# jketterl/digiham

Hardware: AMD Instinct MI355X
Metric: concurrent 48 kS/s DMR channels sustained end-to-end (rrc_filter->gfsk_demodulator->dmr_decoder) (higher is better)
Workload: dtype f32; 1 GPU; 16384 DMR channels/GPU x 3.96 s (190080 samples) of 48 kS/s FM-discriminator audio, full chain rrc(wide)->gfsk(10)->dmr_decoder incl. BPTC(196,96) (BASELINE con; channels_per_gpu=16384, total_channels=16384

## Files before the change

digiham_amd/csrc/dh_portable.hpp:

```cpp
#pragma once

#include <stdint.h>
#include <stddef.h>

#if defined(__HIPCC__) || defined(__HIP__)
#include <hip/hip_runtime.h>
#define DH_DEVICE_BUILD 1
#define DH_HD __host__ __device__ __forceinline__
#define DH_D __device__ __forceinline__
#else
#define DH_DEVICE_BUILD 0
#define DH_HD inline
#define DH_D inline
#endif

#if DH_DEVICE_BUILD && defined(__HIP_DEVICE_COMPILE__)
#define DH_ON_GPU 1
#else
#define DH_ON_GPU 0
#endif

#if DH_ON_GPU
#define DH_GPU_ELSE(gpu, cpu) gpu
#else
#define DH_GPU_ELSE(gpu, cpu) cpu
#endif

#define DH_WAVE 64

#if DH_ON_GPU
static __device__ __forceinline__ int dh_fresh_lane_id_() { int l = (int) threadIdx.x; asm volatile("" : "+v"(l)); return l; }
#define DH_FOR_LANES(lane) for (int lane = (int) threadIdx.x, dh_once_ = 1; dh_once_; dh_once_ = 0)
#define DH_FOR_LANES_FRESH(lane) for (int lane = dh_fresh_lane_id_(), dh_once_ = 1; dh_once_; dh_once_ = 0)
#define DH_BARRIER() do { __builtin_amdgcn_fence(__ATOMIC_RELEASE, "workgroup", "local"); __builtin_amdgcn_s_barrier(); \
                          __builtin_amdgcn_fence(__ATOMIC_ACQUIRE, "workgroup", "local"); } while (0)
#define DH_BALLOT_ACC(mask, pred, lane) (mask) = __builtin_amdgcn_ballot_w64((bool) (pred))
#else
#define DH_FOR_LANES(lane) for (int lane = 0; lane < DH_WAVE; ++lane)
#define DH_FOR_LANES_FRESH(lane) DH_FOR_LANES(lane)
#define DH_BARRIER() ((void) 0)
#define DH_BALLOT_ACC(mask, pred, lane) (mask) |= ((uint64_t) ((pred) ? 1 : 0) << (lane))
#endif
#define DH_IS_LANE0(lane) ((lane) == 0)
DH_HD bool dh_is_writer_lane() { return DH_GPU_ELSE(threadIdx.x == 0, true); }

DH_HD uint32_t dh_uniform(uint32_t x) { return DH_GPU_ELSE((uint32_t) __builtin_amdgcn_readfirstlane((int) x), x); }

DH_HD uint32_t dh_agent_load(const uint32_t* p) { return DH_GPU_ELSE(__hip_atomic_load(p, __ATOMIC_RELAXED, __HIP_MEMORY_SCOPE_AGENT), *p); }
DH_HD bool dh_agent_cas(uint32_t* p, uint32_t& seen, uint32_t want) {
#if DH_ON_GPU
    return __hip_atomic_compare_exchange_strong(p, &seen, want, __ATOMIC_RELAXED, __ATOMIC_RELAXED, __HIP_MEMORY_SCOPE_AGENT);
#else
    if (*p == seen) { *p = want; return true; }
    seen = *p;
    return false;
#endif
}
DH_HD void dh_agent_add(uint32_t* p, uint32_t v) { DH_GPU_ELSE(__hip_atomic_fetch_add(p, v, __ATOMIC_RELAXED, __HIP_MEMORY_SCOPE_AGENT), *p += v); }
DH_HD uint32_t dh_xcc_id() { return DH_GPU_ELSE(__builtin_amdgcn_s_getreg((31 << 11) | 20) & 15u, 0u); }
#if DH_ON_GPU
__device__ __forceinline__ void dh_nap() { __builtin_amdgcn_s_sleep(64); }
__device__ __forceinline__ void dh_acquire_behind_flag() { __builtin_amdgcn_fence(__ATOMIC_ACQUIRE, "agent"); __builtin_amdgcn_s_dcache_inv(); }
__device__ __forceinline__ void dh_release_before_flag() { asm volatile("s_waitcnt vmcnt(0) lgkmcnt(0)" ::: "memory"); __builtin_amdgcn_fence(__ATOMIC_RELEASE, "workgroup"); }
__device__ __forceinline__ uint32_t dh_opaque_scalar(uint32_t x) { asm volatile("" : "+s"(x)); return x; }
__device__ __forceinline__ void dh_barrier_global() { __syncthreads(); }
#else
inline void dh_nap() {}
inline void dh_acquire_behind_flag() {}
inline void dh_release_before_flag() {}
inline uint32_t dh_opaque_scalar(uint32_t x) { return x; }
inline void dh_barrier_global() {}
#endif

DH_HD int dh_popc32(uint32_t x) { return DH_GPU_ELSE(__popc(x), __builtin_popcount(x)); }
DH_HD int dh_popc64(uint64_t x) { return DH_GPU_ELSE(__popcll(x), __builtin_popcountll(x)); }
// ... 179 lines not shown
```

digiham_amd/csrc/dsp_core.hpp:

```cpp
#pragma once

#include "dh_portable.hpp"
#include "wave_ops.hpp"

#define DH_VARIANCE_SYMBOLS 100
#define DH_VOLUME_RB_SIZE 100
#define DH_FTILE 1024
#define DH_FIR_L 16
#define DH_PF_N 5
#define DH_PF_SINK 512
#define DH_MAX_NZ 160
#define DH_MAX_SPS 40
DH_HD uint32_t dh_history(uint32_t sps) { return DH_VARIANCE_SYMBOLS * (sps > 10u ? sps : 10u) + 152u; }
DH_HD uint32_t dh_tail_max(uint32_t sps) { return 256u + dh_history(sps); }
#define DH_STATE_HDR 32

enum { DH_ST_K = 0, DH_ST_OFF = 1, DH_ST_TAIL = 2, DH_ST_NSYM = 3, DH_ST_ORDERED = 4, DH_ST_BLOCKS = 5,
       DH_ST_P0 = 6,
       DH_ST_CUR_START = 7, DH_ST_CUR_OFF = 8, DH_ST_PREV_START = 9, DH_ST_PREV_OFF = 10,
       DH_ST_BLOCK_FLAGS = 11,
       DH_ST_E_CUR = 12, DH_ST_E_PREV = 13, DH_ST_E_COUNT = 14, DH_ST_E_BLOCK = 15,
       DH_ST_UNCERTAIN = 16, DH_ST_EXACT_RUNS = 17, DH_ST_EXACT_BLOCKS = 18,
       DH_ST_PART = 19,
       DH_ST_DIAG = 20 };
// ... 353 lines not shown
    return ok;
}
inline float dh_f16_error_coefficient(const DhF16Taps& F, uint32_t nz, double gain) {
    const double u = 5.9604644775390625e-08;
    const double ks = (double) F.ksteps, nref = 2.0 + (double) nz;
    const double mfma = F.one_chain ? 82.0 * ks * F.l1_g1 * (1.0 + 1.0 / 2048.0) + 41.0 * ks / 2048.0 * (3.0 * F.l1_g2 * (1.0 + 1.0 / 2048.0) + F.l1_g1)
                                    : 41.0 * ks * F.l1_g1 * (1.0 + 1.0 / 2048.0) + 82.0 * ks / 2048.0 * (F.l1_g2 + 0.5 * F.l1_g1);
    const double kl1 = (nref + 0.01) * F.l1 + 1.0001 * F.l1 + mfma
                     + 2.0 * (0.5 * F.l1_g2 / 4194304.0 + F.sum_delta * (1.0 + 1.0 / 4096.0) + u * F.l1) / u + (F.one_chain ? 2.1 : 3.1) * F.l1;
    const double coef = 1.44 * kl1 * u / (gain < 0 ? -gain : gain) * 1.0001;
    float f = (float) coef;
    if ((double) f < coef) { union { float f; uint32_t u; } b; b.f = f; b.u++; f = b.f; }
    return f;
}

#if DH_ON_GPU
template <int NZ, bool ONE>
__device__ __forceinline__ void dh_fir_f16(const float* hw, const dh_u4 (&G)[2 * DH_F16_KSTEPS_OF(NZ)], int lane, float k1, float k2, float* out16) {
    constexpr int DH_F16_KSTEPS = DH_F16_KSTEPS_OF(NZ), DH_F16_FRAGS = 2 * DH_F16_KSTEPS, DH_F16_H2_OFFSET = DH_F16_H2_OFFSET_OF(NZ);
    const int m = lane & 15, q = lane >> 4;
    const char* base = reinterpret_cast<const char*>(hw) + 32 * (int) DH_F16_ROW_BLOCK(m) + 16 * q;
    dh_h8 g[DH_F16_FRAGS];
#pragma unroll
    for (int f = 0; f < DH_F16_FRAGS; f++) g[f] = __builtin_bit_cast(dh_h8, G[f]);
#pragma unroll
    for (int TT = 0; TT < 4; TT += 2) {
        dh_h8 a1[2][DH_F16_KSTEPS], a2[2][DH_F16_KSTEPS];
#pragma unroll
        for (int t = 0; t < 2; t++)
#pragma unroll
            for (int s = 0; s < DH_F16_KSTEPS; s++) a1[t][s] = *reinterpret_cast<const dh_h8*>(base + 512 * (TT + t) + 64 * s);
        if constexpr (ONE) {
            dh_f32x4 acc[2] = { { 0.0f, 0.0f, 0.0f, 0.0f }, { 0.0f, 0.0f, 0.0f, 0.0f } };
#pragma unroll
            for (int s = 0; s < DH_F16_KSTEPS; s++)
#pragma unroll
                for (int t = 0; t < 2; t++) acc[t] = __builtin_amdgcn_mfma_f32_16x16x32_f16(a1[t][s], g[DH_F16_KSTEPS + s], acc[t], 0, 0, 0);
#pragma unroll
            for (int s = 0; s < DH_F16_KSTEPS; s++) {
#pragma unroll
                for (int t = 0; t < 2; t++) acc[t] = __builtin_amdgcn_mfma_f32_16x16x32_f16(a1[t][s], g[s], acc[t], 0, 0, 0);
#pragma unroll
                for (int t = 0; t < 2; t++) a2[t][s] = *reinterpret_cast<const dh_h8*>(base + 512 * (TT + t) + 64 * s + 4 * DH_F16_H2_OFFSET);
            }
#pragma unroll
            for (int s = 0; s < DH_F16_KSTEPS; s++)
#pragma unroll
                for (int t = 0; t < 2; t++) acc[t] = __builtin_amdgcn_mfma_f32_16x16x32_f16(a2[t][s], g[s], acc[t], 0, 0, 0);
#pragma unroll
            for (int t = 0; t < 2; t++)
#pragma unroll
                for (int r = 0; r < 4; r++) out16[4 * (TT + t) + r] = acc[t][r] * k1;
            __builtin_amdgcn_sched_group_barrier(0x100, 2 * DH_F16_KSTEPS, 0);
            __builtin_amdgcn_sched_group_barrier(0x008, 2 * DH_F16_KSTEPS, 0);
#pragma unroll
            for (int s = 0; s < DH_F16_KSTEPS; s++) { __builtin_amdgcn_sched_group_barrier(0x008, 2, 0); __builtin_amdgcn_sched_group_barrier(0x100, 2, 0); }
            __builtin_amdgcn_sched_group_barrier(0x008, 2 * DH_F16_KSTEPS, 0);
            (void) k2;
        } else {
            dh_f32x4 mn[2] = { { 0.0f, 0.0f, 0.0f, 0.0f }, { 0.0f, 0.0f, 0.0f, 0.0f } }, sc[2] = { { 0.0f, 0.0f, 0.0f, 0.0f }, { 0.0f, 0.0f, 0.0f, 0.0f } };
#pragma unroll
            for (int s = 0; s < DH_F16_KSTEPS; s++) {
#pragma unroll
                for (int t = 0; t < 2; t++) sc[t] = __builtin_amdgcn_mfma_f32_16x16x32_f16(a1[t][s], g[DH_F16_KSTEPS + s], sc[t], 0, 0, 0);
#pragma unroll
                for (int t = 0; t < 2; t++) mn[t] = __builtin_amdgcn_mfma_f32_16x16x32_f16(a1[t][s], g[s], mn[t], 0, 0, 0);
#pragma unroll
                for (int t = 0; t < 2; t++) a2[t][s] = *reinterpret_cast<const dh_h8*>(base + 512 * (TT + t) + 64 * s + 4 * DH_F16_H2_OFFSET);
            }
#pragma unroll
            for (int s = 0; s < DH_F16_KSTEPS; s++)
#pragma unroll
                for (int t = 0; t < 2; t++) sc[t] = __builtin_amdgcn_mfma_f32_16x16x32_f16(a2[t][s], g[s], sc[t], 0, 0, 0);
#pragma unroll
            for (int t = 0; t < 2; t++)
#pragma unroll
                for (int r = 0; r < 4; r++) out16[4 * (TT + t) + r] = __builtin_fmaf(sc[t][r], k2, mn[t][r] * k1);
// ... 17 lines not shown
        for (int i = 0; i < 3; i++) {
            const int pass = ONE ? (i == 0 ? 1 : i == 1 ? 0 : 2) : i;
            for (int s = 0; s < DH_F16_KSTEPS; s++) for (int qq = 0; qq < 4; qq++) for (int j = 0; j < 8; j++) {
                const int kk = 8 * qq + j;
                const uint32_t w = G[(pass == 1 ? DH_F16_KSTEPS : 0) + s][16 * qq + n][j >> 1];
                const float tap = dh_f16_value((uint16_t) (w >> (16 * (j & 1))));
                const uint16_t hv = (pass == 2 ? h2 : h1)[b16 + 32u * (uint32_t) s + (uint32_t) kk];
                if (pass == 0 && !ONE) mn = __builtin_fmaf(dh_f16_value(hv), tap, mn); else sc = __builtin_fmaf(dh_f16_value(hv), tap, sc);
            }
        }
        out16[4 * T + r] = ONE ? sc * k1 : __builtin_fmaf(sc, k2, mn * k1);
    }
}
#endif

DH_HD float dh_virtual_sample(const float* tail, uint32_t tc, const float* in, uint32_t idx) {
    return idx < tc ? tail[idx] : in[idx - tc];
}

struct DhAgcPair { float mn0, mx0, mn1, mx1; };

#if DH_ON_GPU
__device__ __forceinline__ void dh_agc_scan(DhDspShared& S, uint32_t k0, uint32_t k1, DH_LANE_STRUCT_REF(DhAgcPair, agc)) {
    const int lane = dh_fresh_lane_id_();
    const uint32_t e0 = 2u * (uint32_t) lane, e1 = e0 + 1u;
    const float c0 = e0 < k0 ? S.vol_old[e0] : S.vol_new[e0];
    const float c1 = e1 < k0 ? S.vol_old[e1] : S.vol_new[e1];
    const bool v0 = e0 < k1, v1 = e1 < k1;
    const float pmn0 = v0 ? c0 : DH_FLT_MAX, pmn1 = v1 ? c1 : DH_FLT_MAX;
    const float pmx0 = v0 ? c0 : DH_FLT_MIN, pmx1 = v1 ? c1 : DH_FLT_MIN;
    float pmn = dh_vmin(pmn0, pmn1), pmx = dh_vmax(pmx0, pmx1);
    const uint32_t r0 = 126u - e0, r1 = r0 + 1u;
    const float o0 = S.vol_old[r0], o1 = S.vol_old[r1];
    const float omn0 = r0 < DH_VOLUME_RB_SIZE ? o0 : DH_FLT_MAX, omn1 = r1 < DH_VOLUME_RB_SIZE ? o1 : DH_FLT_MAX;
    const float omx0 = r0 < DH_VOLUME_RB_SIZE ? o0 : DH_FLT_MIN, omx1 = r1 < DH_VOLUME_RB_SIZE ? o1 : DH_FLT_MIN;
    float smn = dh_vmin(omn0, omn1), smx = dh_vmax(omx0, omx1);
    dh_wave_prefix_minmax2(pmn, pmx, smn, smx);
    float epmn = DH_FLT_MAX, epmx = DH_FLT_MIN, esmn = DH_FLT_MAX, esmx = DH_FLT_MIN;
    dh_wave_prev4(epmn, epmx, esmn, esmx, pmn, pmx, smn, smx);
    const int from = (63 - lane) << 2;
    const float s1n = __int_as_float(__builtin_amdgcn_ds_bpermute(from, __float_as_int(esmn)));
    const float s1x = __int_as_float(__builtin_amdgcn_ds_bpermute(from, __float_as_int(esmx)));
    const float s0n = __int_as_float(__builtin_amdgcn_ds_bpermute(from, __float_as_int(dh_vmin(omn1, esmn))));
    const float s0x = __int_as_float(__builtin_amdgcn_ds_bpermute(from, __float_as_int(dh_vmax(omx1, esmx))));
    DhAgcPair r;
    r.mn0 = dh_vmin(dh_vmin(epmn, pmn0), s0n); r.mx0 = dh_vmax(dh_vmax(epmx, pmx0), s0x);
    r.mn1 = dh_vmin(pmn, s1n); r.mx1 = dh_vmax(pmx, s1x);
    S.mn[e0] = r.mn0; S.mx[e0] = r.mx0; S.mn[e1] = r.mn1; S.mx[e1] = r.mx1;
    agc = r;
}
#else
inline void dh_agc_scan(DhDspShared& S, uint32_t k0, uint32_t k1, DH_LANE_STRUCT_REF(DhAgcPair, agc)) {
    float pmn = DH_FLT_MAX, pmx = DH_FLT_MIN;
    for (uint32_t j = 0; j < k0; j++) { pmn = dh_fmin_(pmn, S.vol_old[j]); pmx = dh_fmax_(pmx, S.vol_old[j]); }
    for (uint32_t k = k0; k < k1; k++) {
        pmn = dh_fmin_(pmn, S.vol_new[k]); pmx = dh_fmax_(pmx, S.vol_new[k]);
        float smn = DH_FLT_MAX, smx = DH_FLT_MIN;
        for (uint32_t j = k + 1; j < DH_VOLUME_RB_SIZE; j++) { smn = dh_fmin_(smn, S.vol_old[j]); smx = dh_fmax_(smx, S.vol_old[j]); }
        S.mn[k] = dh_fmin_(pmn, smn); S.mx[k] = dh_fmax_(pmx, smx);
    }
    for (uint32_t l = 0; l < DH_WAVE; l++) {
        const uint32_t e0 = 2u * l, e1 = e0 + 1u, a = e0 >= k0 && e0 < k1 ? e0 : k0, b = e1 >= k0 && e1 < k1 ? e1 : k0;
        agc[l] = DhAgcPair{ S.mn[a], S.mx[a], S.mn[b], S.mx[b] };
    }
}
#endif

template <int NZ, bool FAST, int SPS> struct DhIsBounded {
// ... 211 lines not shown
                        const uint32_t c = e / nj;
                        jj = e - c * nj;
                        uint64_t m = rows & all;
                        for (uint32_t b = 0; b < c; b++) m &= m - 1;
                        i = (uint32_t) dh_ffs64(m);
                    }
                    const uint32_t j = j0 + jj;
                    const int32_t f = C.cur_start + (int32_t) (j * sps) + (j ? C.cur_off : 0) + (int32_t) i;
                    S.var_rb[i * DH_VARIANCE_SYMBOLS + j] = dh_exact_filtered_lds<NZ>(stage, base, C.nv, C.tapsf, C.gain, C.rgain, f);
                }
            }
        }
    }
    DH_BARRIER();
}

template <int NZ>
DH_COLD void dh_exact_fir_pass(const DhDspParams& P, DhDspShared& S, uint32_t need, DH_LANE_ARRAY(float, (&fo), DH_FIR_L)) {
    float tv[NZ / 2 + 1];
    for (int i = 0; i <= NZ / 2; i++) tv[i] = S.tapsf[i];
    DH_FOR_LANES_FRESH(lane) {
        if ((uint32_t) (lane * DH_FIR_L) < need) {
            dh_fir_lane<NZ, false, false, true>(tv, P.gain, P.rgain, P.inv_gain, S.xf, lane, DH_LA(fo, lane));
        }
    }
}

template <int SPS>
DH_HD void dh_symbol_windows(DhDspShared& S, const float* fbuf, uint32_t k0, uint32_t m, int32_t step_off, uint32_t sps, uint32_t ev_lo, uint32_t ev_hi, float sps_rcp) {
#define DH_FB(n) fbuf[n]
    if (SPS == 10 && DH_STOP_AFTER >= 3) DH_FOR_LANES_FRESH(lane) {
        const uint32_t l = (uint32_t) lane;
        const uint32_t qa = l + 1u, qb = l < 35u ? l + 65u : 0u;
        const bool va = qa < m, vb = l < 35u ? qb < m : l == 35u;
        const float* srca = fbuf + (int32_t) (qa * 10u) + step_off;
        const float* srcb = l < 35u ? srca + 640 : fbuf;
        float v[10], w[10];
        dh_lds_run10_pair(srca, srcb, v, w);
        float vola = v[0], volb = w[0];
#pragma unroll
        for (int i = 1; i < 10; i++) { vola += v[i]; volb += w[i]; }
        const float mida = ((v[3] + v[4]) + v[5]) + v[6], midb = ((w[3] + w[4]) + w[5]) + w[6];
        const float volume_a = dh_div_const(vola, 10.0f, sps_rcp), volume_b = dh_div_const(volb, 10.0f, sps_rcp);
        if (va) {
            const uint32_t ka = k0 + qa;
            dh_lds_store_row10<0>(S.var_rb + ka, v[0], v[1], v[2], v[3], v[4], v[5], v[6], v[7], v[8], v[9]);
            S.sum[qa] = mida; S.vol_new[ka] = volume_a;
        }
        if (vb) {
            const uint32_t kb = k0 + qb;
            dh_lds_store_row10<0>(S.var_rb + kb, w[0], w[1], w[2], w[3], w[4], w[5], w[6], w[7], w[8], w[9]);
            S.sum[qb] = midb; S.vol_new[kb] = volume_b;
        }
        dh_lds_stores_done();
    }
    if (SPS == 20 && DH_STOP_AFTER >= 3) DH_FOR_LANES_FRESH(lane) {
        const uint32_t l = (uint32_t) lane;
        const uint32_t q = l < 63u ? l + 1u : 0u;
        const bool valid = q < m;
        const float* src = valid && q > 0u ? fbuf + (int32_t) (q * 20u) + step_off : fbuf;
        float v[20];
        dh_lds_run<20>(src, v);
        float vol = v[0];
#pragma unroll
        for (int i = 1; i < 20; i++) vol += v[i];
        const float mid = ((((v[7] + v[8]) + v[9]) + v[10]) + v[11]) + v[12];
        const float volume = dh_div_const(vol, 20.0f, sps_rcp);
        if (valid) {
            const uint32_t k = k0 + q;
            dh_lds_store_row10<0>(S.var_rb + k, v[0], v[1], v[2], v[3], v[4], v[5], v[6], v[7], v[8], v[9]);
            dh_lds_store_row10<1000>(S.var_rb + k, v[10], v[11], v[12], v[13], v[14], v[15], v[16], v[17], v[18], v[19]);
            S.sum[q] = mid; S.vol_new[k] = volume;
        }
        dh_lds_stores_done();
    }
    if (SPS == 40 && DH_STOP_AFTER >= 3) DH_FOR_LANES_FRESH(lane) {
// ... 30 lines not shown
                    float value[4];
#pragma unroll
                    for (uint32_t j = 0; j < 4u; j++) value[j] = DH_FB(s + i + j);
#pragma unroll
                    for (uint32_t j = 0; j < 4u; j++) {
                        if (i + j >= ev_lo && i + j < ev_hi) sum += value[j];
                        volume_sum += value[j];
                        S.var_rb[(i + j) * DH_VARIANCE_SYMBOLS + k] = value[j];
                    }
                }
                for (; i < sps; i++) {
                    const float value = DH_FB(s + i);
                    if (i >= ev_lo && i < ev_hi) sum += value;
                    volume_sum += value;
                    S.var_rb[i * DH_VARIANCE_SYMBOLS + k] = value;
                }
            }
            S.sum[q] = sum;
            S.vol_new[k] = dh_div_const(volume_sum, (float) sps, sps_rcp);
        }
    }
#undef DH_FB
}

struct DhStreamView { const float* tail; uint32_t tc; const float* in; uint32_t nv; float sps_rcp; };
template <int NZ, int SPS, bool BOUNDED>
DH_HD int32_t dh_timing_decision(const DhDspParams& P, DhDspShared& S, DhBoundState* const BS, const DhStreamView& V, uint32_t sps, uint32_t k0, float e_blk) {
    const float* const tail = V.tail; const uint32_t tc = V.tc; const float* const in = V.in; const uint32_t nv = V.nv; const float sps_rcp = V.sps_rcp;
    int32_t new_off = 0;
    {
        bool ordered = true;
        uint64_t chain_rows = ~0ull;
        bool est_done = false;
        if (SPS == 10 && !P.ordered_timing) {
            DH_LANE_ARRAY(float, gs, 1); DH_LANE_ARRAY(float, gq, 1);
            DH_FOR_LANES_FRESH(lane) {
                const uint32_t r = (uint32_t) lane >> 4, c = (uint32_t) lane & 15u;
                const uint32_t j = (c * 205u) >> 10, g = c - 5u * j, i = 3u * r + j;
                const bool act = c < 15u && i < 10u;
                const dh_f4a* row = reinterpret_cast<const dh_f4a*>(S.var_rb + (act ? i * DH_VARIANCE_SYMBOLS + g * 20u : 0u));
                dh_f2 s2 = dh_f2_make(0.0f, 0.0f), q2 = dh_f2_make(0.0f, 0.0f);
#pragma unroll
                for (int q = 0; q < 5; q++) {
                    const dh_f4a v = row[q];
                    const dh_f2 a = dh_f2_make(v.x, v.y), b = dh_f2_make(v.z, v.w);
                    s2 = dh_f2_add(s2, a); s2 = dh_f2_add(s2, b);
                    q2 = dh_f2_fma(a, a, q2); q2 = dh_f2_fma(b, b, q2);
                }
                DH_LA(gs, lane)[0] = act ? s2.x + s2.y : 0.0f; DH_LA(gq, lane)[0] = act ? q2.x + q2.y : 0.0f;
            }
            DH_LANE_ARRAY(float, lo, 1); DH_LANE_ARRAY(float, hi, 1);
            uint64_t vote_above = 0, fine_cand = 0, fine_out = 0;
            dh_row_sum5_pair(gs, gq);
            DH_FOR_LANES_FRESH(lane) {
                const uint32_t r = (uint32_t) lane >> 4, c = (uint32_t) lane & 15u;
                const bool own = (((r == 3u ? 0x0010u : 0x4210u) >> c) & 1u) != 0u;
                const float total = DH_LA(gs, lane)[0], e = DH_LA(gq, lane)[0] * 0.01f;
                const float mean = total * 0.01f;
                const float v = __builtin_fmaf(-mean, mean, e);
                float tol = __builtin_fmaf(e, 4e-6f, 1e-42f);
                if (BOUNDED && e_blk > 0.0f) tol += 8.0f * e_blk * dh_sqrt_upper(__builtin_fmaxf(v, 0.0f) + 4.0f * e_blk * e_blk) + 8.0f * e_blk * e_blk;
                const float l = own ? v - tol : DH_FLT_MAX, h = own ? v + tol : DH_FLT_MAX;
                DH_LA(lo, lane)[0] = l; DH_LA(hi, lane)[0] = h;
                const bool sane = e < 1e30f && v != 0.0f;
                DH_BALLOT_ACC(fine_cand, !own || (sane && l > 0.0f && h < 4999999.0f), lane);
                DH_BALLOT_ACC(fine_out, !own || sane, lane);
            }
            const float hmin = DH_WAVE_MIN(hi);
            DH_FOR_LANES_FRESH(lane) {
                DH_BALLOT_ACC(vote_above, DH_LA(lo, lane)[0] > hmin, lane);
            }
            const uint64_t cand = ~vote_above;
            const uint64_t unfit = (vote_above & ~fine_out) | (cand & ~fine_cand);
            if (DH_LIKELY((unfit | (cand & (cand - 1))) == 0 && cand != 0)) {
                est_done = true; ordered = false;
                constexpr uint64_t UP = (1ull << 9) | (1ull << 14) | (1ull << 20) | (1ull << 25), DOWN = (1ull << 30) | (1ull << 36) | (1ull << 41) | (1ull << 46);
                new_off = (cand & UP) ? +1 : (cand & DOWN) ? -1 : 0;
            }
        }
        if (SPS == 10 && !P.ordered_timing && !est_done) {
            DH_BARRIER();
            float* psum = S.mn; float* pd = S.mx;
            DH_FOR_LANES_FRESH(lane) {
                if (lane < 50) {
                    const uint32_t i = ((uint32_t) lane * 205u) >> 10, g = (uint32_t) lane - 5u * i;
                    const uint32_t ro = i * DH_VARIANCE_SYMBOLS + g * 20u;
                    const dh_f4a* row = reinterpret_cast<const dh_f4a*>(S.var_rb + ro);
                    dh_f2 s2 = dh_f2_make(0.0f, 0.0f), q2 = dh_f2_make(0.0f, 0.0f);
#pragma unroll
                    for (int q = 0; q < 5; q++) {
                        const dh_f4a v = row[q];
                        const dh_f2 a = dh_f2_make(v.x, v.y), b = dh_f2_make(v.z, v.w);
                        s2 = dh_f2_add(s2, a); s2 = dh_f2_add(s2, b);
                        q2 = dh_f2_fma(a, a, q2); q2 = dh_f2_fma(b, b, q2);
                    }
                    psum[lane] = s2.x + s2.y; pd[lane] = q2.x + q2.y;
                }
            }
            DH_BARRIER();
            DH_LANE_ARRAY(float, lo, 1); DH_LANE_ARRAY(float, hi, 1);
            uint64_t vote_guard = 0, vote_vzero = 0, vote_zero = 0, vote_pos = 0, vote_small = 0, vote_above = 0;
            DH_FOR_LANES_FRESH(lane) {
                float l = DH_FLT_MAX, h = DH_FLT_MAX;
                bool guard = true, vzero = false;
                if (lane < 10) {
                    const int i = lane;
                    const float total = (((psum[5 * i] + psum[5 * i + 1]) + psum[5 * i + 2]) + psum[5 * i + 3]) + psum[5 * i + 4];
                    const float e = ((((pd[5 * i] + pd[5 * i + 1]) + pd[5 * i + 2]) + pd[5 * i + 3]) + pd[5 * i + 4]) * 0.01f;
                    const float mean = total * 0.01f;
                    const float v = __builtin_fmaf(-mean, mean, e);
                    float tol = __builtin_fmaf(e, 4e-6f, 1e-42f);
                    if (BOUNDED && e_blk > 0.0f) tol += 8.0f * e_blk * dh_sqrt_upper(__builtin_fmaxf(v, 0.0f) + 4.0f * e_blk * e_blk) + 8.0f * e_blk * e_blk;
                    guard = e < 1e30f;
// ... 715 lines not shown
        const float T_eff = force_doubt ? __builtin_inff() : T;
        const float inv_width = 1.0f / (float) (ev_hi - ev_lo);
        const bool width_pow2 = ((ev_hi - ev_lo) & (ev_hi - ev_lo - 1u)) == 0u;
        const bool pair_store = ((uint32_t) (uintptr_t) syms + nsym) % 2u == 0u;

        dh_symbol_windows<SPS>(S, fbuf, k0, m, step_off, sps, ev_lo, ev_hi, sps_rcp);
        DH_BARRIER();
        DH_PHASE_MARK(2);

        dh_issue_next_window<NZ, PF_REG>(S, in, tc, p_next, pf_plain, pf_reg, pfr);

        DH_LANE_STRUCT(DhAgcPair, agc) = {};
        if (DH_STOP_AFTER >= 4) dh_agc_scan(S, k0, k0 + m, agc);
        DH_BARRIER();
        DH_PHASE_MARK(3);

        if (DH_STOP_AFTER >= 5) {
            const DhSliceSetup U = { four_levels, e_pos, width_pow2, pair_store, T_eff, inv_width };
            dh_slice_symbols<SPS, LV, BOUNDED>(P, S, agc, syms + nsym, k0, m, ev_lo, ev_hi, U, vote_a, vote_b);
        }
        if (BOUNDED && DH_UNLIKELY((vote_a | vote_b) != 0)) {
            dh_settle_doubts<NZ>(P, S, BS, V, syms + nsym, k0, e_eff, sps, ev_lo, ev_hi, vote_a, vote_b);
        }

        DH_PHASE_MARK(4);
        int32_t new_off = 0;
        const bool block_done = (k0 + m == DH_VARIANCE_SYMBOLS);
        if (block_done && DH_STOP_AFTER >= 6) {
            new_off = dh_timing_decision<NZ, SPS, BOUNDED>(P, S, BS, V, sps, k0, e_blk);
        }

        DH_PHASE_MARK(5);
        DH_FOR_LANES_FRESH(lane) {
            const uint32_t ka = k0 + (uint32_t) lane, kb = ka + DH_WAVE, ke = k0 + m;
            const uint32_t ia = ka < ke ? ka : k0, ib = kb < ke ? kb : k0;
            const float va_ = S.vol_new[ia], vb_ = S.vol_new[ib];
            S.vol_old[ia] = va_;
            S.vol_old[ib] = vb_;
        }
        staged_p = 0xFFFFFFFFu;
        if (DH_LIKELY(pf_reg)) {
            if constexpr (PF_REG && MF16) { if (DH_LIKELY((dh_stage_f16<NZ, ONE_CHAIN>(P, S, pfr, pf_have, st_e_run, st_k1, st_k2)))) staged_p = p_next; }
            else if constexpr (PF_PLAIN) {
                static_assert(!PF_PLAIN || (DH_FTILE == 4u * DH_WAVE * (DH_PF_N - 1)), "four full groups cover the window");
                DH_FOR_LANES_FRESH(lane) {
                    const uint32_t l4 = 4u * (uint32_t) lane;
                    float* ldst = &S.xf[l4];
#pragma unroll
                    for (int r = 0; r < DH_PF_N - 1; r++) {
                        dh_f4 w = DH_LA(pfr, lane)[PF_REG ? r : 0];
                        if (DH_UNLIKELY(pf_have < DH_FTILE)) w = dh_zero_beyond(w, l4 + 4u * DH_WAVE * (uint32_t) r, pf_have);
                        dh_store4(ldst + 4 * DH_WAVE * r, w);
                    }
                }
                staged_p = p_next;
            }
        }
        DH_BARRIER();
        p = p_next;
        nsym += m;
        if (k0 == 0) off = 0;
        k0 += m;
        if (block_done) { k0 = 0; off = new_off; }
        if (BOUNDED) {
            const float ec = dh_uniform_f(__builtin_fmaxf(e_cur, e_run));
            const uint32_t cnt = e_count + m;
            if (cnt >= DH_VOLUME_RB_SIZE) { e_prev = ec; e_cur = 0.0f; e_count = 0; }
            else { e_cur = ec; e_count = cnt; }
// ... 169 lines not shown
```

digiham_amd/csrc/wave_ops.hpp:

```cpp
#pragma once

#include "dh_portable.hpp"

#define DH_FLT_MAX 3.402823466e+38f
#define DH_DBL_MAX 1.7976931348623157e+308
#define DH_FLT_MIN 1.175494351e-38f

#if DH_ON_GPU
typedef float dh_f2 __attribute__((ext_vector_type(2)));
typedef float dh_v4f __attribute__((ext_vector_type(4)));
typedef float dh_f32x4 __attribute__((ext_vector_type(4)));
typedef _Float16 dh_h8 __attribute__((ext_vector_type(8)));
typedef _Float16 dh_h4 __attribute__((ext_vector_type(4)));
typedef uint32_t dh_u4 __attribute__((ext_vector_type(4)));
#else
struct dh_f2 { float x, y; };
typedef uint16_t dh_h4[4];
#endif
struct __attribute__((aligned(4))) dh_f4 { float x, y, z, w; };
struct alignas(16) dh_f4a { float x, y, z, w; };
DH_HD dh_f4 dh_load4_unaligned(const float* p) { dh_f4 v; __builtin_memcpy(&v, p, sizeof(v)); return v; }
DH_HD void dh_store4(float* q, const dh_f4& v) { q[0] = v.x; q[1] = v.y; q[2] = v.z; q[3] = v.w; }
DH_HD void dh_store4_unaligned(float* q, const dh_f4& v) { __builtin_memcpy(q, &v, sizeof(v)); }

// ... 32 lines not shown
    else           asm("v_pk_mul_f32 %0, %1, %2 op_sel:[1,0] op_sel_hi:[1,1]" : "=v"(p) : "s"(cc), "v"(w));
    return acc + p;
}
#endif

DH_HD float dh_mul_uniform(float s, float v) {
#if DH_ON_GPU
    float r; asm("v_mul_f32 %0, %1, %2" : "=v"(r) : "s"(s), "v"(v)); return r;
#else
    return v * s;
#endif
}

DH_HD float dh_div_const(float x, float d, float r) {
    union { float f; uint32_t u; } a; a.f = x;
    const uint32_t t = (a.u << 1) - 2u * 0x0D800000u;
    if (t > 2u * (0x71800000u - 0x0D800000u)) return x / d;
    const float q0 = x * r;
    const float rem = __builtin_fmaf(-q0, d, x);
    return __builtin_fmaf(rem, r, q0);
}
#if DH_ON_GPU
__device__ __forceinline__ dh_f2 dh_div_const2(dh_f2 x, float d, float r) {
    const uint32_t ta = (__float_as_uint(x.x) << 1) - 2u * 0x0D800000u, tb = (__float_as_uint(x.y) << 1) - 2u * 0x0D800000u;
    if (__builtin_expect((ta > tb ? ta : tb) > 2u * (0x71800000u - 0x0D800000u), 0)) { dh_f2 q; q.x = dh_div_const(x.x, d, r); q.y = dh_div_const(x.y, d, r); return q; }
    const dh_f2 rr = { r, r }, dd = { -d, -d };
    const dh_f2 q0 = x * rr;
    const dh_f2 rem = __builtin_elementwise_fma(q0, dd, x);
    return __builtin_elementwise_fma(rem, rr, q0);
}
#else
inline dh_f2 dh_div_const2(dh_f2 x, float d, float r) { return dh_f2_make(dh_div_const(x.x, d, r), dh_div_const(x.y, d, r)); }
#endif

DH_HD float dh_sqrt_upper(float x) {
    const float a = x > 1e-30f ? x : 1e-30f;
    return DH_GPU_ELSE(__builtin_amdgcn_sqrtf(a), __builtin_sqrtf(a)) * 1.00000095367431640625f;
}

DH_HD float dh_fmin_(float a, float b) { return b < a ? b : a; }
DH_HD float dh_fmax_(float a, float b) { return b > a ? b : a; }
#if DH_ON_GPU
__device__ __forceinline__ float dh_vmin(float a, float b) { float r; asm("v_min_f32 %0, %1, %2" : "=v"(r) : "v"(a), "v"(b)); return r; }
__device__ __forceinline__ float dh_vmax(float a, float b) { float r; asm("v_max_f32 %0, %1, %2" : "=v"(r) : "v"(a), "v"(b)); return r; }
__device__ __forceinline__ float dh_min3_abs(float a, float b, float c) { float r; asm("v_min3_f32 %0, |%1|, |%2|, |%3|" : "=v"(r) : "v"(a), "v"(b), "v"(c)); return r; }
__device__ __forceinline__ float dh_max3_abs(float a, float b, float c) { float r; asm("v_maximum3_f32 %0, |%1|, |%2|, %3" : "=v"(r) : "v"(a), "v"(b), "v"(c)); return r; }
#else
inline float dh_vmin(float a, float b) { return __builtin_fminf(a, b); }
inline float dh_vmax(float a, float b) { return __builtin_fmaxf(a, b); }
inline float dh_min3_abs(float a, float b, float c) { return __builtin_fminf(__builtin_fminf(__builtin_fabsf(a), __builtin_fabsf(b)), __builtin_fabsf(c)); }
inline float dh_max3_abs(float a, float b, float c) {
    if (a != a || b != b || c != c) return __builtin_nanf("");
    return __builtin_fmaxf(c, __builtin_fmaxf(__builtin_fabsf(a), __builtin_fabsf(b)));
}
#endif
template <int N> DH_HD float dh_max_abs_groups(const dh_f4 (&w)[N]) {
#if DH_ON_GPU
    static_assert(N == 5, "five groups of four");
    float mx;
    const dh_f4 w0 = w[0], w1 = w[1], w2 = w[2], w3 = w[3], w4 = w[4];
    asm("v_maximum3_f32 %0, |%1|, |%2|, 0\n\tv_maximum3_f32 %0, |%3|, |%4|, %0\n\tv_maximum3_f32 %0, |%5|, |%6|, %0\n\tv_maximum3_f32 %0, |%7|, |%8|, %0\n\t"
        "v_maximum3_f32 %0, |%9|, |%10|, %0\n\tv_maximum3_f32 %0, |%11|, |%12|, %0\n\tv_maximum3_f32 %0, |%13|, |%14|, %0\n\tv_maximum3_f32 %0, |%15|, |%16|, %0\n\t"
        "v_maximum3_f32 %0, |%17|, |%18|, %0\n\tv_maximum3_f32 %0, |%19|, |%20|, %0"
        : "=&v"(mx) : "v"(w0.x), "v"(w0.y), "v"(w0.z), "v"(w0.w), "v"(w1.x), "v"(w1.y), "v"(w1.z), "v"(w1.w), "v"(w2.x), "v"(w2.y), "v"(w2.z), "v"(w2.w),
                      "v"(w3.x), "v"(w3.y), "v"(w3.z), "v"(w3.w), "v"(w4.x), "v"(w4.y), "v"(w4.z), "v"(w4.w));
    return mx;
// ... 126 lines not shown
__device__ __forceinline__ void dh_lds_stores_done() { asm volatile("s_waitcnt lgkmcnt(0)" ::: "memory"); }
template <int K> __device__ __forceinline__ void dh_lds_store_row10(float* base, float a0, float a1, float a2, float a3, float a4, float a5, float a6, float a7, float a8, float a9) {
    const uint32_t addr = (uint32_t) (uintptr_t) (__attribute__((address_space(3))) float*) base;
    asm volatile("ds_write_b32 %0, %1 offset:%11\n\tds_write_b32 %0, %2 offset:%12\n\tds_write_b32 %0, %3 offset:%13\n\tds_write_b32 %0, %4 offset:%14\n\t"
                 "ds_write_b32 %0, %5 offset:%15\n\tds_write_b32 %0, %6 offset:%16\n\tds_write_b32 %0, %7 offset:%17\n\tds_write_b32 %0, %8 offset:%18\n\t"
                 "ds_write_b32 %0, %9 offset:%19\n\tds_write_b32 %0, %10 offset:%20"
                 :: "v"(addr), "v"(a0), "v"(a1), "v"(a2), "v"(a3), "v"(a4), "v"(a5), "v"(a6), "v"(a7), "v"(a8), "v"(a9),
                    "n"(4 * K), "n"(4 * (K + 100)), "n"(4 * (K + 200)), "n"(4 * (K + 300)), "n"(4 * (K + 400)), "n"(4 * (K + 500)), "n"(4 * (K + 600)),
                    "n"(4 * (K + 700)), "n"(4 * (K + 800)), "n"(4 * (K + 900)) : "memory");
}
#else
template <int OFF_WORDS> inline void dh_lds_store4_at(float* base, const dh_f4& v) { dh_store4(base + OFF_WORDS, v); }
inline void dh_lds_stores_done() {}
template <int K> inline void dh_lds_store_row10(float* base, float a0, float a1, float a2, float a3, float a4, float a5, float a6, float a7, float a8, float a9) {
    const float a[10] = { a0, a1, a2, a3, a4, a5, a6, a7, a8, a9 };
    for (int i = 0; i < 10; i++) base[i * 100 + K] = a[i];
}
#endif

DH_HD void dh_l2_touch_lines(const float* base, uint32_t n, float* sink) {
#if DH_ON_GPU
    const uint32_t pf_lane = (uint32_t) dh_fresh_lane_id_();
    const float* line = base + 32u * pf_lane;
    const uint32_t sink_addr = (uint32_t) (uintptr_t) (__attribute__((address_space(3))) float*) sink;
    uint32_t keep_m0;
    if (32u * pf_lane < n)
        asm volatile("s_mov_b32 %0, m0\n\ts_mov_b32 m0, %1\n\tglobal_load_lds_dword %2, off\n\ts_mov_b32 m0, %0"
                     : "=&s"(keep_m0) : "s"(sink_addr), "v"(line) : "memory");
#endif
}
DH_HD void dh_global_loads_done() { DH_GPU_ELSE(asm volatile("s_waitcnt vmcnt(0)" ::: "memory"), (void) 0); }

#if DH_ON_GPU
#define DH_TAPFRAG_REGS(name, N, table) dh_u4 name[N]
#define DH_TAPFRAG_LOAD(name, N, table, on) do { if constexpr (on) { const dh_u4* tf_ = reinterpret_cast<const dh_u4*>(table) + dh_fresh_lane_id_(); \
        _Pragma("unroll") for (int f_ = 0; f_ < (N); f_++) name[f_] = tf_[DH_WAVE * f_]; } } while (0)
#define DH_TAPFRAG_SETTLE(name, N, on) do { if constexpr (on) { _Pragma("unroll") for (int f_ = 0; f_ < (N); f_++) \
        asm volatile("" :: "v"(name[f_])); } } while (0)
#else
#define DH_TAPFRAG_REGS(name, N, table) const uint32_t (* const name)[DH_WAVE][4] = reinterpret_cast<const uint32_t (*)[DH_WAVE][4]>(table)
#define DH_TAPFRAG_LOAD(name, N, table, on) ((void) 0)
#define DH_TAPFRAG_SETTLE(name, N, on) ((void) 0)
#endif

#if DH_ON_GPU
__device__ __forceinline__ void dh_wave_prefix_minmax2(float& mn, float& mx, float& mn2, float& mx2) {
#define DH_SCAN_STEP4(ctrl) \
    "v_min_f32_dpp %0, %0, %0 " ctrl "\n\tv_max_f32_dpp %1, %1, %1 " ctrl "\n\tv_min_f32_dpp %2, %2, %2 " ctrl "\n\tv_max_f32_dpp %3, %3, %3 " ctrl "\n\t"
    asm volatile("s_nop 4\n\t"
                 DH_SCAN_STEP4("row_shr:1 row_mask:0xf bank_mask:0xf")
                 DH_SCAN_STEP4("row_shr:2 row_mask:0xf bank_mask:0xf")
                 DH_SCAN_STEP4("row_shr:4 row_mask:0xf bank_mask:0xf")
                 DH_SCAN_STEP4("row_shr:8 row_mask:0xf bank_mask:0xf")
                 DH_SCAN_STEP4("row_bcast:15 row_mask:0xa bank_mask:0xf")
                 DH_SCAN_STEP4("row_bcast:31 row_mask:0xc bank_mask:0xf")
                 "s_nop 1"
                 : "+v"(mn), "+v"(mx), "+v"(mn2), "+v"(mx2));
#undef DH_SCAN_STEP4
}
__device__ __forceinline__ void dh_wave_prev4(float& a, float& b, float& c, float& d, float va, float vb, float vc, float vd) {
    asm volatile("s_nop 4\n\tv_mov_b32_dpp %0, %4 wave_shr:1 row_mask:0xf bank_mask:0xf\n\tv_mov_b32_dpp %1, %5 wave_shr:1 row_mask:0xf bank_mask:0xf\n\t"
                 "v_mov_b32_dpp %2, %6 wave_shr:1 row_mask:0xf bank_mask:0xf\n\tv_mov_b32_dpp %3, %7 wave_shr:1 row_mask:0xf bank_mask:0xf\n\ts_nop 1"
                 : "+v"(a), "+v"(b), "+v"(c), "+v"(d) : "v"(va), "v"(vb), "v"(vc), "v"(vd));
}

__device__ __forceinline__ float dh_wave_max(float v) {
#define DH_MAX_STEP(ctrl) "s_nop 1\n\tv_max_f32_dpp %0, %0, %0 " ctrl "\n\t"
    asm volatile("s_nop 4\n\t"
                 DH_MAX_STEP("row_shr:1 row_mask:0xf bank_mask:0xf") DH_MAX_STEP("row_shr:2 row_mask:0xf bank_mask:0xf")
                 DH_MAX_STEP("row_shr:4 row_mask:0xf bank_mask:0xf") DH_MAX_STEP("row_shr:8 row_mask:0xf bank_mask:0xf")
                 DH_MAX_STEP("row_bcast:15 row_mask:0xa bank_mask:0xf") DH_MAX_STEP("row_bcast:31 row_mask:0xc bank_mask:0xf")
                 "s_nop 1" : "+v"(v));
#undef DH_MAX_STEP
    return __int_as_float(__builtin_amdgcn_readlane(__float_as_int(v), 63));
}
__device__ __forceinline__ float dh_wave_max_nan(float f) {
    uint32_t v = __float_as_uint(f);
#define DH_MAX_STEP(ctrl) "s_nop 1\n\tv_max_u32_dpp %0, %0, %0 " ctrl "\n\t"
    asm volatile("s_nop 4\n\t"
                 DH_MAX_STEP("row_shr:1 row_mask:0xf bank_mask:0xf") DH_MAX_STEP("row_shr:2 row_mask:0xf bank_mask:0xf")
                 DH_MAX_STEP("row_shr:4 row_mask:0xf bank_mask:0xf") DH_MAX_STEP("row_shr:8 row_mask:0xf bank_mask:0xf")
                 DH_MAX_STEP("row_bcast:15 row_mask:0xa bank_mask:0xf") DH_MAX_STEP("row_bcast:31 row_mask:0xc bank_mask:0xf")
                 "s_nop 1" : "+v"(v));
#undef DH_MAX_STEP
    return __int_as_float(__builtin_amdgcn_readlane((int) v, 63));
}
__device__ __forceinline__ float dh_row_min_to_lane15(float v) {
    asm volatile("s_nop 4\n\tv_min_f32_dpp %0, %0, %0 row_shr:1 row_mask:0xf bank_mask:0xf\n\t"
                 "s_nop 1\n\tv_min_f32_dpp %0, %0, %0 row_shr:2 row_mask:0xf bank_mask:0xf\n\t"
                 "s_nop 1\n\tv_min_f32_dpp %0, %0, %0 row_shr:4 row_mask:0xf bank_mask:0xf\n\t"
                 "s_nop 1\n\tv_min_f32_dpp %0, %0, %0 row_shr:8 row_mask:0xf bank_mask:0xf\n\ts_nop 1"
                 : "+v"(v));
    return __int_as_float(__builtin_amdgcn_readlane(__float_as_int(v), 15));
}
#else
inline float dh_wave_max_lanes(const float (&a)[DH_WAVE][1]) {
    float m = 0.0f;
    for (int l = 0; l < DH_WAVE; l++) m = __builtin_fmaxf(m, a[l][0]);
    return m;
}
inline float dh_wave_max_nan_lanes(const float (&a)[DH_WAVE][1]) {
    uint32_t m = 0;
    for (int l = 0; l < DH_WAVE; l++) { union { float f; uint32_t u; } b; b.f = a[l][0]; if (b.u > m) m = b.u; }
    union { float f; uint32_t u; } r; r.u = m;
    return r.f;
}
inline float dh_wave_min_lanes(const float (&a)[DH_WAVE][1], int lanes) {
    float m = DH_FLT_MAX;
    for (int l = 0; l < lanes; l++) m = dh_fmin_(m, a[l][0]);
    return m;
}
#endif
#if DH_ON_GPU
#define DH_WAVE_MAX(a) dh_wave_max((a)[0])
#define DH_WAVE_MAX_NAN(a) dh_wave_max_nan((a)[0])
#define DH_WAVE_MIN(a) (-dh_wave_max(-(a)[0]))
#define DH_ROW0_MIN(a) dh_row_min_to_lane15((a)[0])
#else
#define DH_WAVE_MAX(a) dh_wave_max_lanes(a)
#define DH_WAVE_MAX_NAN(a) dh_wave_max_nan_lanes(a)
#define DH_WAVE_MIN(a) dh_wave_min_lanes(a, DH_WAVE)
#define DH_ROW0_MIN(a) dh_wave_min_lanes(a, 16)
#endif

// ... 25 lines not shown
```

Baseline: 14.26 million channels.

## Micro-tune lane predicates, DPP nops, paired division and MFMA operand settling

New measurement: 14.29 million channels, median of 5. About the same (+0.2%).

```diff
diff --git a/digiham_amd/csrc/dh_portable.hpp b/digiham_amd/csrc/dh_portable.hpp
--- a/digiham_amd/csrc/dh_portable.hpp
+++ b/digiham_amd/csrc/dh_portable.hpp
@@ -41,6 +41,7 @@
 #define DH_BARRIER() ((void) 0)
 #define DH_BALLOT_ACC(mask, pred, lane) (mask) |= ((uint64_t) ((pred) ? 1 : 0) << (lane))
 #endif
+#define DH_LANE_IN(mask, lane) DH_GPU_ELSE(__builtin_amdgcn_inverse_ballot_w64((uint64_t) (mask)), ((((uint64_t) (mask)) >> (lane)) & 1ull) != 0ull)
 #define DH_IS_LANE0(lane) ((lane) == 0)
 DH_HD bool dh_is_writer_lane() { return DH_GPU_ELSE(threadIdx.x == 0, true); }
 
diff --git a/digiham_amd/csrc/dsp_core.hpp b/digiham_amd/csrc/dsp_core.hpp
--- a/digiham_amd/csrc/dsp_core.hpp
+++ b/digiham_amd/csrc/dsp_core.hpp
@@ -409,6 +409,8 @@
             for (int s = 0; s < DH_F16_KSTEPS; s++) a1[t][s] = *reinterpret_cast<const dh_h8*>(base + 512 * (TT + t) + 64 * s);
         if constexpr (ONE) {
             dh_f32x4 acc[2] = { { 0.0f, 0.0f, 0.0f, 0.0f }, { 0.0f, 0.0f, 0.0f, 0.0f } };
+            static_assert(DH_F16_KSTEPS == 3, "one chain: the wide filter, six fragments per group");
+            dh_lds_settle6(a1[0][0], a1[1][0], a1[0][1], a1[1][1], a1[0][2], a1[1][2]);
 #pragma unroll
             for (int s = 0; s < DH_F16_KSTEPS; s++)
 #pragma unroll
@@ -420,6 +422,7 @@
 #pragma unroll
                 for (int t = 0; t < 2; t++) a2[t][s] = *reinterpret_cast<const dh_h8*>(base + 512 * (TT + t) + 64 * s + 4 * DH_F16_H2_OFFSET);
             }
+            dh_lds_settle6(a2[0][0], a2[1][0], a2[0][1], a2[1][1], a2[0][2], a2[1][2]);
 #pragma unroll
             for (int s = 0; s < DH_F16_KSTEPS; s++)
 #pragma unroll
@@ -503,8 +506,10 @@
     float pmn = dh_vmin(pmn0, pmn1), pmx = dh_vmax(pmx0, pmx1);
     const uint32_t r0 = 126u - e0, r1 = r0 + 1u;
     const float o0 = S.vol_old[r0], o1 = S.vol_old[r1];
-    const float omn0 = r0 < DH_VOLUME_RB_SIZE ? o0 : DH_FLT_MAX, omn1 = r1 < DH_VOLUME_RB_SIZE ? o1 : DH_FLT_MAX;
-    const float omx0 = r0 < DH_VOLUME_RB_SIZE ? o0 : DH_FLT_MIN, omx1 = r1 < DH_VOLUME_RB_SIZE ? o1 : DH_FLT_MIN;
+    static_assert(DH_VOLUME_RB_SIZE == 100, "lanes 14 .. 63");
+    const bool in_ring = DH_LANE_IN(~0x3FFFull, lane);
+    const float omn0 = in_ring ? o0 : DH_FLT_MAX, omn1 = in_ring ? o1 : DH_FLT_MAX;
+    const float omx0 = in_ring ? o0 : DH_FLT_MIN, omx1 = in_ring ? o1 : DH_FLT_MIN;
     float smn = dh_vmin(omn0, omn1), smx = dh_vmax(omx0, omx1);
     dh_wave_prefix_minmax2(pmn, pmx, smn, smx);
     float epmn = DH_FLT_MAX, epmx = DH_FLT_MIN, esmn = DH_FLT_MAX, esmx = DH_FLT_MIN;
@@ -782,7 +787,8 @@
     if (SPS == 10 && DH_STOP_AFTER >= 3) DH_FOR_LANES_FRESH(lane) {
         const uint32_t l = (uint32_t) lane;
         const uint32_t qa = l + 1u, qb = l < 35u ? l + 65u : 0u;
-        const bool va = qa < m, vb = l < 35u ? qb < m : l == 35u;
+        const uint32_t nb = m > 65u ? m - 65u : 0u;
+        const bool va = qa < m, vb = l < nb || l == 35u;
         const float* srca = fbuf + (int32_t) (qa * 10u) + step_off;
         const float* srcb = l < 35u ? srca + 640 : fbuf;
         float v[10], w[10];
@@ -791,7 +797,8 @@
 #pragma unroll
         for (int i = 1; i < 10; i++) { vola += v[i]; volb += w[i]; }
         const float mida = ((v[3] + v[4]) + v[5]) + v[6], midb = ((w[3] + w[4]) + w[5]) + w[6];
-        const float volume_a = dh_div_const(vola, 10.0f, sps_rcp), volume_b = dh_div_const(volb, 10.0f, sps_rcp);
+        float volume_a, volume_b;
+        dh_div_const_both(vola, volb, 10.0f, sps_rcp, volume_a, volume_b);
         if (va) {
             const uint32_t ka = k0 + qa;
             dh_lds_store_row10<0>(S.var_rb + ka, v[0], v[1], v[2], v[3], v[4], v[5], v[6], v[7], v[8], v[9]);
@@ -888,13 +895,13 @@
         bool ordered = true;
         uint64_t chain_rows = ~0ull;
         bool est_done = false;
-        if (SPS == 10 && !P.ordered_timing) {
+        if (SPS == 10 && DH_LIKELY(!P.ordered_timing)) {
             DH_LANE_ARRAY(float, gs, 1); DH_LANE_ARRAY(float, gq, 1);
             DH_FOR_LANES_FRESH(lane) {
-                const uint32_t r = (uint32_t) lane >> 4, c = (uint32_t) lane & 15u;
-                const uint32_t j = (c * 205u) >> 10, g = c - 5u * j, i = 3u * r + j;
-                const bool act = c < 15u && i < 10u;
-                const dh_f4a* row = reinterpret_cast<const dh_f4a*>(S.var_rb + (act ? i * DH_VARIANCE_SYMBOLS + g * 20u : 0u));
+                constexpr uint64_t ACT = 0x001F7FFF7FFF7FFFull;
+                static_assert(DH_VARIANCE_SYMBOLS == 100, "300 r + 20 c");
+                const bool act = DH_LANE_IN(ACT, lane);
+                const dh_f4a* row = reinterpret_cast<const dh_f4a*>(S.var_rb + (act ? 20u * ((uint32_t) lane - ((uint32_t) lane >> 4)) : 0u));
                 dh_f2 s2 = dh_f2_make(0.0f, 0.0f), q2 = dh_f2_make(0.0f, 0.0f);
 #pragma unroll
                 for (int q = 0; q < 5; q++) {
@@ -909,13 +916,13 @@
             uint64_t vote_above = 0, fine_cand = 0, fine_out = 0;
             dh_row_sum5_pair(gs, gq);
             DH_FOR_LANES_FRESH(lane) {
-                const uint32_t r = (uint32_t) lane >> 4, c = (uint32_t) lane & 15u;
-                const bool own = (((r == 3u ? 0x0010u : 0x4210u) >> c) & 1u) != 0u;
+                constexpr uint64_t OWN = 0x0010421042104210ull;
+                const bool own = DH_LANE_IN(OWN, lane);
                 const float total = DH_LA(gs, lane)[0], e = DH_LA(gq, lane)[0] * 0.01f;
                 const float mean = total * 0.01f;
                 const float v = __builtin_fmaf(-mean, mean, e);
                 float tol = __builtin_fmaf(e, 4e-6f, 1e-42f);
-                if (BOUNDED && e_blk > 0.0f) tol += 8.0f * e_blk * dh_sqrt_upper(__builtin_fmaxf(v, 0.0f) + 4.0f * e_blk * e_blk) + 8.0f * e_blk * e_blk;
+                if (BOUNDED) tol += 8.0f * e_blk * dh_sqrt_upper(__builtin_fmaxf(v, 0.0f) + 4.0f * e_blk * e_blk) + 8.0f * e_blk * e_blk;
                 const float l = own ? v - tol : DH_FLT_MAX, h = own ? v + tol : DH_FLT_MAX;
                 DH_LA(lo, lane)[0] = l; DH_LA(hi, lane)[0] = h;
                 const bool sane = e < 1e30f && v != 0.0f;
@@ -934,7 +941,7 @@
                 new_off = (cand & UP) ? +1 : (cand & DOWN) ? -1 : 0;
             }
         }
-        if (SPS == 10 && !P.ordered_timing && !est_done) {
+        if (SPS == 10 && !P.ordered_timing && DH_UNLIKELY(!est_done)) {
             DH_BARRIER();
             float* psum = S.mn; float* pd = S.mx;
             DH_FOR_LANES_FRESH(lane) {
@@ -1716,8 +1723,8 @@
 
         DH_PHASE_MARK(5);
         DH_FOR_LANES_FRESH(lane) {
-            const uint32_t ka = k0 + (uint32_t) lane, kb = ka + DH_WAVE, ke = k0 + m;
-            const uint32_t ia = ka < ke ? ka : k0, ib = kb < ke ? kb : k0;
+            const uint32_t ka = k0 + (uint32_t) lane, kb = ka + DH_WAVE, kl = k0 + m - 1u;
+            const uint32_t ia = dh_min<uint32_t>(ka, kl), ib = dh_min<uint32_t>(kb, kl);
             const float va_ = S.vol_new[ia], vb_ = S.vol_new[ib];
             S.vol_old[ia] = va_;
             S.vol_old[ib] = vb_;
diff --git a/digiham_amd/csrc/wave_ops.hpp b/digiham_amd/csrc/wave_ops.hpp
--- a/digiham_amd/csrc/wave_ops.hpp
+++ b/digiham_amd/csrc/wave_ops.hpp
@@ -88,6 +88,17 @@
 #else
 inline dh_f2 dh_div_const2(dh_f2 x, float d, float r) { return dh_f2_make(dh_div_const(x.x, d, r), dh_div_const(x.y, d, r)); }
 #endif
+DH_HD void dh_div_const_both(float xa, float xb, float d, float r, float& qa, float& qb) {
+#if DH_ON_GPU
+    const uint32_t ta = (__float_as_uint(xa) << 1) - 2u * 0x0D800000u, tb = (__float_as_uint(xb) << 1) - 2u * 0x0D800000u;
+    if (__builtin_expect(__builtin_amdgcn_ballot_w64((ta > tb ? ta : tb) > 2u * (0x71800000u - 0x0D800000u)) != 0, 0)) { qa = xa / d; qb = xb / d; return; }
+    const float a0 = xa * r, b0 = xb * r;
+    const float ra = __builtin_fmaf(-a0, d, xa), rb = __builtin_fmaf(-b0, d, xb);
+    qa = __builtin_fmaf(ra, r, a0); qb = __builtin_fmaf(rb, r, b0);
+#else
+    qa = dh_div_const(xa, d, r); qb = dh_div_const(xb, d, r);
+#endif
+}
 
 DH_HD float dh_sqrt_upper(float x) {
     const float a = x > 1e-30f ? x : 1e-30f;
@@ -280,11 +291,15 @@
 DH_HD void dh_global_loads_done() { DH_GPU_ELSE(asm volatile("s_waitcnt vmcnt(0)" ::: "memory"), (void) 0); }
 
 #if DH_ON_GPU
+template <typename T> __device__ __forceinline__ void dh_lds_settle6(T& a, T& b, T& c, T& d, T& e, T& f) {
+    asm("" : "+v"(a), "+v"(b), "+v"(c), "+v"(d), "+v"(e), "+v"(f));
+}
 #define DH_TAPFRAG_REGS(name, N, table) dh_u4 name[N]
 #define DH_TAPFRAG_LOAD(name, N, table, on) do { if constexpr (on) { const dh_u4* tf_ = reinterpret_cast<const dh_u4*>(table) + dh_fresh_lane_id_(); \
         _Pragma("unroll") for (int f_ = 0; f_ < (N); f_++) name[f_] = tf_[DH_WAVE * f_]; } } while (0)
-#define DH_TAPFRAG_SETTLE(name, N, on) do { if constexpr (on) { _Pragma("unroll") for (int f_ = 0; f_ < (N); f_++) \
-        asm volatile("" :: "v"(name[f_])); } } while (0)
+#define DH_TAPFRAG_SETTLE(name, N, on) do { if constexpr (on) { static_assert((N) % 6 == 0, "six fragments per statement"); \
+        _Pragma("unroll") for (int f_ = 0; f_ < (N); f_ += 6) \
+        asm volatile("" :: "v"(name[f_]), "v"(name[f_ + 1]), "v"(name[f_ + 2]), "v"(name[f_ + 3]), "v"(name[f_ + 4]), "v"(name[f_ + 5])); } } while (0)
 #else
 #define DH_TAPFRAG_REGS(name, N, table) const uint32_t (* const name)[DH_WAVE][4] = reinterpret_cast<const uint32_t (*)[DH_WAVE][4]>(table)
 #define DH_TAPFRAG_LOAD(name, N, table, on) ((void) 0)
@@ -313,23 +328,23 @@
 }
 
 __device__ __forceinline__ float dh_wave_max(float v) {
-#define DH_MAX_STEP(ctrl) "s_nop 1\n\tv_max_f32_dpp %0, %0, %0 " ctrl "\n\t"
+#define DH_MAX_STEP(ctrl) "v_max_f32_dpp %0, %0, %0 " ctrl
     asm volatile("s_nop 4\n\t"
-                 DH_MAX_STEP("row_shr:1 row_mask:0xf bank_mask:0xf") DH_MAX_STEP("row_shr:2 row_mask:0xf bank_mask:0xf")
-                 DH_MAX_STEP("row_shr:4 row_mask:0xf bank_mask:0xf") DH_MAX_STEP("row_shr:8 row_mask:0xf bank_mask:0xf")
-                 DH_MAX_STEP("row_bcast:15 row_mask:0xa bank_mask:0xf") DH_MAX_STEP("row_bcast:31 row_mask:0xc bank_mask:0xf")
-                 "s_nop 1" : "+v"(v));
+                 DH_MAX_STEP("row_shr:1 row_mask:0xf bank_mask:0xf") "\n\ts_nop 1\n\t" DH_MAX_STEP("row_shr:2 row_mask:0xf bank_mask:0xf") "\n\ts_nop 1\n\t"
+                 DH_MAX_STEP("row_shr:4 row_mask:0xf bank_mask:0xf") "\n\ts_nop 1\n\t" DH_MAX_STEP("row_shr:8 row_mask:0xf bank_mask:0xf") "\n\ts_nop 1\n\t"
+                 DH_MAX_STEP("row_bcast:15 row_mask:0xa bank_mask:0xf") "\n\ts_nop 1\n\t" DH_MAX_STEP("row_bcast:31 row_mask:0xc bank_mask:0xf")
+                 : "+v"(v));
 #undef DH_MAX_STEP
     return __int_as_float(__builtin_amdgcn_readlane(__float_as_int(v), 63));
 }
 __device__ __forceinline__ float dh_wave_max_nan(float f) {
     uint32_t v = __float_as_uint(f);
-#define DH_MAX_STEP(ctrl) "s_nop 1\n\tv_max_u32_dpp %0, %0, %0 " ctrl "\n\t"
+#define DH_MAX_STEP(ctrl) "v_max_u32_dpp %0, %0, %0 " ctrl
     asm volatile("s_nop 4\n\t"
-                 DH_MAX_STEP("row_shr:1 row_mask:0xf bank_mask:0xf") DH_MAX_STEP("row_shr:2 row_mask:0xf bank_mask:0xf")
-                 DH_MAX_STEP("row_shr:4 row_mask:0xf bank_mask:0xf") DH_MAX_STEP("row_shr:8 row_mask:0xf bank_mask:0xf")
-                 DH_MAX_STEP("row_bcast:15 row_mask:0xa bank_mask:0xf") DH_MAX_STEP("row_bcast:31 row_mask:0xc bank_mask:0xf")
-                 "s_nop 1" : "+v"(v));
+                 DH_MAX_STEP("row_shr:1 row_mask:0xf bank_mask:0xf") "\n\ts_nop 1\n\t" DH_MAX_STEP("row_shr:2 row_mask:0xf bank_mask:0xf") "\n\ts_nop 1\n\t"
+                 DH_MAX_STEP("row_shr:4 row_mask:0xf bank_mask:0xf") "\n\ts_nop 1\n\t" DH_MAX_STEP("row_shr:8 row_mask:0xf bank_mask:0xf") "\n\ts_nop 1\n\t"
+                 DH_MAX_STEP("row_bcast:15 row_mask:0xa bank_mask:0xf") "\n\ts_nop 1\n\t" DH_MAX_STEP("row_bcast:31 row_mask:0xc bank_mask:0xf")
+                 : "+v"(v));
 #undef DH_MAX_STEP
     return __int_as_float(__builtin_amdgcn_readlane((int) v, 63));
 }
@@ -337,7 +352,7 @@
     asm volatile("s_nop 4\n\tv_min_f32_dpp %0, %0, %0 row_shr:1 row_mask:0xf bank_mask:0xf\n\t"
                  "s_nop 1\n\tv_min_f32_dpp %0, %0, %0 row_shr:2 row_mask:0xf bank_mask:0xf\n\t"
                  "s_nop 1\n\tv_min_f32_dpp %0, %0, %0 row_shr:4 row_mask:0xf bank_mask:0xf\n\t"
-                 "s_nop 1\n\tv_min_f32_dpp %0, %0, %0 row_shr:8 row_mask:0xf bank_mask:0xf\n\ts_nop 1"
+                 "s_nop 1\n\tv_min_f32_dpp %0, %0, %0 row_shr:8 row_mask:0xf bank_mask:0xf"
                  : "+v"(v));
     return __int_as_float(__builtin_amdgcn_readlane(__float_as_int(v), 15));
 }
```
